# 2noise/ChatTTS

Measured on AMD Instinct MI355X. Metric: audio seconds/sec (RTF), batch=64 per GPU, higher is better.
Workload: dtype f32x3

## Files before the change

### chattts_amd/_lib.py

```python
from __future__ import annotations

import ctypes as C
import os

import torch

HERE = os.path.dirname(os.path.abspath(__file__))
LIB_PATH = os.environ.get("CTTS_LIB") or os.path.join(HERE, "csrc", "libchattts_amd.so")

F32, BF16 = 0, 1
P = C.c_void_p
PP = C.POINTER(C.c_void_p)


class GptWeights(C.Structure):
    _fields_ = [
        ("n_layers", C.c_int32), ("weight_dtype", C.c_int32), ("kv_dtype", C.c_int32), ("max_pos", C.c_int32),
        ("wqkv", PP), ("wo", PP), ("wgu", PP), ("wd", PP), ("ln1", PP), ("ln2", PP),
        ("norm", P), ("emb_code", P), ("heads", P), ("rope_cos", P), ("rope_sin", P),
        ("rms_eps", C.c_float),
        ("emb_text", P), ("head_text", P), ("n_text", C.c_int32),
        ("wqkv_pk", PP), ("wo_pk", PP), ("wgu_pk", PP), ("wd_pk", PP),
        ("heads_pk", P), ("head_text_pk", P),
        ("wo_hd", PP),
# ... 105 lines not shown
    "ctts_k_gemm": (C.c_int, [I32, P, P, P, I32, I32, I32, I32, I32, I32, I32, P, F, P, I32, P, P, I32, I32, I32, I32, I32, P]),
    "ctts_k_gemm_x3p": (C.c_int, [P, P, I32, I32, I32, I32, P, P, P, P, P, P]),
    "ctts_k_gemm_h1p": (C.c_int, [P, P, I32, I32, I32, I32, P, P, P, P, P, P]),
    "ctts_stream_create_cu_mask": (C.c_int, [I32, I32, I32, I32, P]),
    "ctts_stream_destroy": (C.c_int, [P]),
    "ctts_k_mlp_fused": (C.c_int, [P, P, P, I32, I32, P, P, P, P, I32, P]),
    "ctts_k_gemm_fast": (C.c_int, [P, I32, P, I32, I32, I32, P, F, I32, P, I32, P, I32, P, P]),
    "ctts_k_qkv_rope": (C.c_int, [P, P, I32, P, F, P, P, P, I32, P, P, I32, P, P, I32, P]),
    "ctts_k_gemm_dec": (C.c_int, [P, P, I32, I32, I32, P, P, F, I32, P, I32, P, I32, P, I32, P]),
    "ctts_k_gemm_dec32x": (C.c_int, [P, C.c_int64, P, C.c_int64, I32, I32, I32, P, P, I32, F, I32, P, I32, P, I32, P, C.c_int64, I32, P, I32, P, P, P]),
    "ctts_k_gemm_pre_x3": (C.c_int, [P, I32, P, P, I32, I32, I32, I32, I32, P, P, P, I32, P]),
    "ctts_k_dec32_last_variant": (C.c_char_p, []),
    "ctts_k_gemm_dec32": (C.c_int, [P, P, I32, I32, I32, P, P, I32, P, F, I32, P, I32, P, I32, P, I32, I32, I32, P]),
    "ctts_k_rows_prep": (C.c_int, [P, P, P, I32, P]),
    "ctts_k_rope_append": (C.c_int, [P, P, P, I32, I32, P, P, I32, P, P, I32, P]),
    "ctts_k_attention": (C.c_int, [P, P, P, I32, I32, P, I32, P, P, I32, P]),
    "ctts_k_attention_prefill": (C.c_int, [P, P, P, I32, P, I32, I32, P, I32, P]),
    "ctts_k_attention_dec": (C.c_int, [P, P, P, I32, P, P, P, I32, P, P, I32, P]),
    "ctts_k_attention_dec2": (C.c_int, [P, P, P, I32, I32, P, P, P, I32, I32, P]),
    "ctts_k_attention_cfg": (C.c_int, [I32, I32, I32]),
    "ctts_k_attention_heads_per_wg": (C.c_int, [I32]),
    "ctts_rccl_unique_id": (C.c_int, [P]),
    "ctts_rccl_comm_create": (C.c_int, [P, I32, P, I32]),
    "ctts_rccl_comm_destroy": (None, [P]),
    "ctts_broadcast_weights": (C.c_int, [P, P, I32, P, I32, P]),
    "ctts_k_attention_oproj": (C.c_int, [P, P, P, I32, P, P, P, I32, P, P, P, P, P, P]),
    "ctts_k_device_guard_probe": (C.c_int, [P, P, P, P, P]),
    "ctts_k_embed_codes": (C.c_int, [P, P, I32, P, P, I32, P]),
    "ctts_k_final_norm": (C.c_int, [P, I32, P, F, P, P, I32, P, I32, I32, P]),
    "ctts_k_sample": (C.c_int, [C.POINTER(GenState), P, P]),
# ... 44 lines not shown
```

### chattts_amd/csrc/capi.hip

```cpp
#include <hip/hip_runtime.h>
#include <dlfcn.h>
#include <stdarg.h>
#include <stdio.h>
#include <stdlib.h>
#include <string.h>
#include <algorithm>
#include <map>
#include <vector>

#include "../../include/chattts_amd.h"
#include "kernels.hpp"

static thread_local char g_err[512] = "";
int ctts_fail(const char* fmt, ...) {
  va_list ap;
  va_start(ap, fmt);
  vsnprintf(g_err, sizeof(g_err), fmt, ap);
  va_end(ap);
  return -1;
}
#define fail ctts_fail
#define CK(expr)                                                                                   \
  do {                                                                                             \
    hipError_t _e = (expr);                                                                        \
// ... 11 lines not shown
  std::vector<const void*> wqkv_pk, wo_pk, wgu_pk, wd_pk;
  std::vector<const void*> wo_hd;
  std::vector<const void*> wqkv_x3, wo_x3, wgu_x3, wd_x3;
  bool dec_x3 = false;
  bool qkv_att = false;
  bool att_oproj = false;
  bool dec_packed = false;
  bool dec_packed32 = false;
  bool heads_packed = false;
  int pf_mask = 0;
  int temporal_layers = 0;
  bool pre32_packed = true;
  bool embed_fold = false;
  bool pre_compact = true;
  bool pre_x3 = true;
  bool fnorm_fuse = true;
  std::vector<const float*> ln1, ln2;
  hipGraph_t graph = nullptr;
  hipGraphExec_t exec = nullptr;
  hipGraph_t graph_multi = nullptr;
  hipGraphExec_t exec_multi = nullptr;
  struct RowsGraph { hipGraph_t graph = nullptr, gm = nullptr; hipGraphExec_t exec = nullptr, exec_multi = nullptr; };
  std::map<int, RowsGraph> rows_graphs;
  int multi_steps = 1;
  int prof_tag = -1;
  int prof_max = 0;
  bool skip_finished = true;
  int n_cu = 0;
  int prof_stride = 1;
  int prof_seen = 0;
// ... 90 lines not shown
    g->wgu_x3.assign(w->wgu_x3, w->wgu_x3 + L);
    g->wd_x3.assign(w->wd_x3, w->wd_x3 + L);
    g->dec_x3 = true;
  }
  if (w->wo_hd && g->dec_packed) {
    g->wo_hd.assign(w->wo_hd, w->wo_hd + L);
    const char* e = getenv("CTTS_ATT_OPROJ");
    g->att_oproj = e && atoi(e) == 1;
  }
  { const char* e = getenv("CTTS_SKIP_FINISHED"); if (e && atoi(e) == 0) g->skip_finished = false; }
  { const char* e = getenv("CTTS_FNORM_FUSE"); if (e && atoi(e) == 0) g->fnorm_fuse = false; }
  { const char* e = getenv("CTTS_W_TEMPORAL_LAYERS"); if (e) g->temporal_layers = atoi(e); }
  { const char* e = getenv("CTTS_PF"); if (e) g->pf_mask = atoi(e); }
  { const char* e = getenv("CTTS_QKV_ATT"); g->qkv_att = e && atoi(e) == 1; }
  { const char* e = getenv("CTTS_PRE32_PACKED"); if (e && atoi(e) == 0) g->pre32_packed = false; }
  { const char* e = getenv("CTTS_PRE_X3"); if (e && atoi(e) == 0) g->pre_x3 = false; }
  { const char* e = getenv("CTTS_PRE_COMPACT"); if (e && atoi(e) == 0) g->pre_compact = false; }
  { const char* e = getenv("CTTS_EMBED_FOLD"); if (e) g->embed_fold = atoi(e) != 0; }
  {
    int dev = 0, cus = 0;
    const char* e = getenv("CTTS_ATT_SPLIT");
    if (e && atoi(e) == 1 && hipGetDevice(&dev) == hipSuccess &&
        hipDeviceGetAttribute(&cus, hipDeviceAttributeMultiprocessorCount, dev) == hipSuccess && cus > 0 && cus <= ATT_CUS_MAX)
      g->n_cu = cus;
  }
  *out = g;
  return 0;
}

extern "C" void ctts_gpt_graph_destroy(ctts_gpt* g) {
  if (!g) return;
// ... 255 lines not shown
    d.epi = D32_EPI_QKV_ROPE; d.C = ws.qkv; d.ldc = 3 * HID; d.desc = ws.desc; d.cos_t = g->w.rope_cos; d.sin_t = g->w.rope_sin;
    d.kc = (float*)kc; d.vc = (float*)vc; d.cmax = cmax;
    CK(launch_gemm_pre32(d, ws.rstd, st));
    CK(launch_attention(ws.qkv, kc, vc, kt, cmax, ws.aop32, 3, rm, M, st));
    d.Ap = ws.aop32; d.Wp = (const float*)g->wo_pk[l]; d.N = HID; d.norm_w = nullptr; d.epi = EPI_RES; d.C = ws.x; d.ldc = HID;
    d.res = ws.x; d.ldr = HID; d.Cp = ws.xp32; d.kch_out = HID / 16;
    CK(launch_gemm_pre32(d, nullptr, st));
    CK(launch_rows_rstd32(ws.x, HID, M, g->w.rms_eps, ws.rstd, st));
    d.Ap = ws.xp32; d.Wp = (const float*)g->wgu_pk[l]; d.N = INTER; d.norm_w = g->ln2[l]; d.epi = EPI_SILU_MUL; d.C = nullptr;
    d.res = nullptr; d.Cp = ws.actp32; d.kch_out = INTER / 16;
    CK(launch_gemm_pre32(d, ws.rstd, st));
    d.Ap = ws.actp32; d.Wp = (const float*)g->wd_pk[l]; d.N = HID; d.K = INTER; d.norm_w = nullptr; d.epi = EPI_RES;
    d.C = ws.x; d.ldc = HID; d.res = ws.x; d.ldr = HID; d.Cp = ws.xp32; d.kch_out = HID / 16;
    CK(launch_gemm_pre32(d, nullptr, st));
  }
  for (int l = 0; !fast && !packed32 && !pre32 && !x3 && l < g->w.n_layers; ++l) {
    void* kc = (char*)s->kcache + kv_layer * l;
    void* vc = (char*)s->vcache + kv_layer * l;
    GemmArgs a;
    memset(&a, 0, sizeof(a));
    a.taps = 1;
    a.n_active = nact;
    a.A = ws.x; a.lda = HID; a.W = g->wqkv[l]; a.C = ws.qkv; a.ldc = 3 * HID; a.M = M; a.N = 3 * HID; a.K = HID; a.wt = wt;
    a.epi = EPI_STORE; a.norm_w = g->ln1[l]; a.eps = g->w.rms_eps;
    if (pre_x3) { CK(launch_rows_rstd32(ws.x, HID, M, g->w.rms_eps, ws.rstd, st)); CK(launch_gemm_pre_x3(a, ws.rstd, st)); }
    else { Prof p(g, 1, st, prof_ok); CK(launch_gemm_skinny(a, st)); }
    { Prof p(g, 2, st, prof_ok); CK(launch_rope_append(ws.qkv, kc, vc, kt, cmax, g->w.rope_cos, g->w.rope_sin, rm, M, st)); }
    { Prof p(g, 3, st, prof_ok); CK(launch_attention(ws.qkv, kc, vc, kt, cmax, ws.ao, 0, rm, M, st)); }
    a.A = ws.ao; a.lda = HID; a.W = g->wo[l]; a.C = ws.x; a.ldc = HID; a.N = HID; a.K = HID; a.epi = EPI_RES; a.norm_w = nullptr;
    a.res = ws.x; a.ldr = HID;
    if (pre_x3) CK(launch_gemm_pre_x3(a, nullptr, st));
    else { Prof p(g, 4, st, prof_ok); CK(launch_gemm_skinny(a, st)); }
    a.A = ws.x; a.W = g->wgu[l]; a.C = ws.act; a.ldc = INTER; a.N = INTER; a.K = HID; a.epi = EPI_SILU_MUL; a.norm_w = g->ln2[l];
    a.res = nullptr;
    if (pre_x3) { CK(launch_rows_rstd32(ws.x, HID, M, g->w.rms_eps, ws.rstd, st)); CK(launch_gemm_pre_x3(a, ws.rstd, st)); }
    else { Prof p(g, 5, st, prof_ok); CK(launch_gemm_skinny(a, st)); }
    a.A = ws.act; a.lda = INTER; a.W = g->wd[l]; a.C = ws.x; a.ldc = HID; a.N = HID; a.K = INTER; a.epi = EPI_RES; a.norm_w = nullptr;
    a.res = ws.x; a.ldr = HID;
    if (pre_x3) CK(launch_gemm_pre_x3(a, nullptr, st));
    else { Prof p(g, 6, st, prof_ok); CK(launch_gemm_skinny(a, st)); }
  }
  if (!heads) return 0;
  if (fuse_fnorm) {
    const int nlog = s->infer_text ? g->w.n_text : NVQ * NAUDIO;
    Dec32Args d;
    memset(&d, 0, sizeof(d));
    d.Ap = x3 ? ws.hfinp : ws.xp32; d.Wp = s->infer_text ? g->w.head_text_pk : g->w.heads_pk; d.M = Bh; d.N = (nlog + 15) / 16 * 16; d.K = HID; d.n_active = nact;
    d.epi = EPI_STORE; d.C = ws.logits; d.ldc = nlog; d.n_cols = nlog;
    d.fnorm = 1; d.norm_w = g->w.norm; d.eps = g->w.rms_eps; d.desc = ws.desc; d.hid = s->hiddens; d.hid_cap = s->hid_cap ? s->hid_cap : s->max_new;
    d.T = s->T; d.prompt_len = s->prompt_len;
    Prof p(g, 8, st, prof_ok);
    CK(launch_gemm_dec32(d, st));
  } else {
  { Prof p(g, 7, st, prof_ok);
// ... 619 lines not shown
  return 0;
}
extern "C" int ctts_k_rope_append(float* qkv, void* kcache, void* vcache, int32_t kv_dtype, int32_t cmax, const float* cos_tab,
                                  const float* sin_tab, int32_t q_per_b, const int32_t* len, const int32_t* kv_start, int32_t M,
                                  void* stream) {
  GptRowMap rm{q_per_b, len, kv_start, nullptr, nullptr, nullptr, nullptr, nullptr, nullptr, 0, 0, 0};
  CK(launch_rope_append(qkv, kcache, vcache, kv_dtype, cmax, cos_tab, sin_tab, rm, M, (hipStream_t)stream));
  return 0;
}
extern "C" int ctts_k_attention(const float* qkv, const void* kcache, const void* vcache, int32_t kv_dtype, int32_t cmax, float* out,
                                int32_t q_per_b, const int32_t* len, const int32_t* kv_start, int32_t M, void* stream) {
  GptRowMap rm{q_per_b, len, kv_start, nullptr, nullptr, nullptr, nullptr, nullptr, nullptr, 0, 0, 0};
  CK(launch_attention(qkv, kcache, vcache, kv_dtype, cmax, out, 0, rm, M, (hipStream_t)stream));
  return 0;
}
extern "C" int ctts_k_attention_prefill(const float* qkv, const uint16_t* kcache, const uint16_t* vcache, int32_t cmax, float* out, int32_t q_per_b,
                                        int32_t slot0, const int32_t* kv_start, int32_t M, void* stream) {
  GptRowMap rm{q_per_b, nullptr, kv_start, nullptr, nullptr, nullptr, nullptr, nullptr, nullptr, 0, slot0, 0};
  CK(launch_attention(qkv, kcache, vcache, WT_BF16, cmax, out, 0, rm, M, (hipStream_t)stream));
  return 0;
}
extern "C" int ctts_k_attention_dec(const float* qkv, const uint16_t* kcache, const uint16_t* vcache, int32_t cmax, uint16_t* out_packed,
                                    const int32_t* desc, const int32_t* n_active, int32_t M, float* part, int32_t* cnt, int32_t n_cu,
                                    void* stream) {
  if (n_cu < 0 || n_cu > ATT_CUS_MAX) return fail("ctts_k_attention_dec: bad n_cu");
  GptRowMap rm{1, nullptr, nullptr, nullptr, n_active, nullptr, reinterpret_cast<const RowDesc*>(desc), part, cnt, n_cu, 0, 0};
  CK(launch_attention(qkv, kcache, vcache, WT_BF16, cmax, out_packed, 2, rm, M, (hipStream_t)stream));
  return 0;
}
extern "C" int ctts_k_attention_dec2(const float* qkv, const void* kcache, const void* vcache, int32_t kv_dtype, int32_t cmax, void* out_packed,
// ... 30 lines not shown
  CK(launch_embed_codes(emb_code, ids_buf, tcap, len, x, nullptr, nullptr, B, nullptr, nullptr, (hipStream_t)stream));
  return 0;
}
extern "C" int ctts_k_final_norm(const float* x, int32_t q_per_b, const float* w, float eps, float* hfin, float* hiddens,
                                 int32_t max_new, const int32_t* len, int32_t T, int32_t B, void* stream) {
  CK(launch_final_norm(x, q_per_b, w, eps, hfin, hiddens, max_new, len, T, B, nullptr, nullptr, nullptr, (hipStream_t)stream));
  return 0;
}
extern "C" int ctts_k_gemm_pre_x3(const float* A, int32_t lda, const float* W, float* C, int32_t ldc, int32_t M, int32_t N, int32_t K, int32_t epi,
                                  const float* norm_w, const float* rstd, const float* res, int32_t ldr, void* stream) {
  GemmArgs a;
  memset(&a, 0, sizeof(a));
  a.taps = 1; a.A = A; a.lda = lda; a.W = W; a.C = C; a.ldc = ldc; a.M = M; a.N = N; a.K = K; a.wt = WT_F32; a.epi = epi;
  a.norm_w = norm_w; a.res = res; a.ldr = ldr;
  CK(launch_gemm_pre_x3(a, rstd, (hipStream_t)stream));
  return 0;
}
extern "C" int ctts_k_sample(const ctts_gen_state* s, const float* logits, void* stream) {
  if (!s || !logits) return fail("ctts_k_sample: bad arguments");
  CK(launch_sample(make_sample_args(s, logits), (hipStream_t)stream));
  return 0;
}
extern "C" int ctts_k_sample_text(const ctts_gen_state* s, const float* logits, int32_t n_text, void* stream) {
  if (!s || !logits || n_text <= 0 || n_text > NTEXT_MAX) return fail("ctts_k_sample_text: bad arguments");
  CK(launch_sample_text(make_sample_args(s, logits), n_text, (hipStream_t)stream));
  return 0;
}
extern "C" int ctts_k_device_guard_probe(void* stream, int32_t* before, int32_t* stream_dev, int32_t* inside, int32_t* switched) {
  if (!before || !stream_dev || !inside || !switched) return fail("ctts_k_device_guard_probe: null argument");
  int b = -1, in = -1;
// ... 126 lines not shown
```

### chattts_amd/csrc/gpt.hip

```cpp
#include <stdlib.h>

#include "common.hpp"
#include "kernels.hpp"
#include "decode_dev.hpp"

#ifndef CTTS_QF_DELAY
#define CTTS_QF_DELAY 8
#endif
#ifndef CTTS_QF_PRE
#define CTTS_QF_PRE 1
#endif
#define HID 768
#define NHEAD 12
#define HDIM 64
#define NVQ 4
#define NAUDIO 626

__device__ __forceinline__ void row_to_b_slot(const GptRowMap& rm, int m, int& b, int& slot) {
  if (rm.q_per_b == 1) { b = rm.row_map ? rm.row_map[m] : m; slot = rm.len[b] - 1; }
  else { b = m / rm.q_per_b; slot = rm.slot0 + m - b * rm.q_per_b; if (rm.row_map) b = rm.row_map[b]; }
}
__device__ __forceinline__ bool row_absent(const int32_t* n_active, int m) { return n_active != nullptr && m >= *n_active; }

__device__ __forceinline__ void emit_row(float4 s, int t, float* __restrict__ x_row, uint16_t* __restrict__ xb_row,
// ... 231 lines not shown
template <> __device__ __forceinline__ void unpack16<float, 4>(const u128& r, float* f) {
  f[0] = __uint_as_float(r.x); f[1] = __uint_as_float(r.y); f[2] = __uint_as_float(r.z); f[3] = __uint_as_float(r.w);
}
template <> __device__ __forceinline__ void unpack16<bf16_t, 8>(const u128& r, float* f) {
  f[0] = __uint_as_float(r.x << 16); f[1] = __uint_as_float(r.x & 0xffff0000u);
  f[2] = __uint_as_float(r.y << 16); f[3] = __uint_as_float(r.y & 0xffff0000u);
  f[4] = __uint_as_float(r.z << 16); f[5] = __uint_as_float(r.z & 0xffff0000u);
  f[6] = __uint_as_float(r.w << 16); f[7] = __uint_as_float(r.w & 0xffff0000u);
}

template <typename OT> __device__ __forceinline__ size_t pko_off(int m, int c);
template <> __device__ __forceinline__ size_t pko_off<bf16_t>(int m, int c) { return pk_off(m, c, HID / 32); }
template <> __device__ __forceinline__ size_t pko_off<float>(int m, int c) { return pk32_off(m, c, HID / 16); }
struct x3p_t { uint16_t v; };
template <> __device__ __forceinline__ size_t pko_off<x3p_t>(int m, int c) { return pk_off(m, c, HID / 32); }
template <typename OT> __device__ __forceinline__ void store_out(OT* p, float v);
template <> __device__ __forceinline__ void store_out<x3p_t>(x3p_t* p, float v) { p->v = f32_to_bf16(v); }
template <typename OT> __device__ __forceinline__ void store_pko(OT* out, int m, int c, float v, size_t);
template <> __device__ __forceinline__ void store_pko<x3p_t>(x3p_t* out, int m, int c, float v, size_t plane) {
  uint16_t* p = reinterpret_cast<uint16_t*>(out) + pk_off(m, c, HID / 32);
  uint16_t h, l;
  x3_split(v, h, l);
  p[0] = h;
  p[plane] = l;
}
template <> __device__ __forceinline__ void store_out<float>(float* p, float v) { *p = v; }
template <> __device__ __forceinline__ void store_out<bf16_t>(bf16_t* p, float v) { *p = f32_to_bf16(v); }
template <> __device__ __forceinline__ void store_pko<float>(float* out, int m, int c, float v, size_t) { out[pko_off<float>(m, c)] = v; }
template <> __device__ __forceinline__ void store_pko<bf16_t>(bf16_t* out, int m, int c, float v, size_t) { out[pko_off<bf16_t>(m, c)] = f32_to_bf16(v); }

// ... 326 lines not shown
  u128 wv[OPJ ? 3 : 1][OPJ ? 8 : 1];
  if constexpr (OPJ) {
    const u128* wo = reinterpret_cast<const u128*>(rm.wo_h) + (size_t)h * 8 * HID + tid;
#pragma unroll
    for (int jc = 0; jc < 3; ++jc)
#pragma unroll
      for (int g8 = 0; g8 < 8; ++g8) wv[jc][g8] = load16(wo + (size_t)g8 * HID + 256 * jc);
    __builtin_amdgcn_sched_barrier(0);
  }
  lrun = groups_sum<LPK>(lrun, lane);
#pragma unroll
  for (int e = 0; e < DPL; ++e) acc[e] = groups_sum<LPK>(acc[e], lane);
  if (NW == 1) {
    if (kg == 0) {
      const float inv = 1.0f / lrun;
      OT* op = PKO ? out + pko_off<OT>(m, h * HDIM + dl * DPL) : out + (size_t)m * HID + h * HDIM + dl * DPL;
#pragma unroll
      for (int e = 0; e < DPL; ++e) store_out<OT>(op + e, acc[e] * inv);
    }
    return;
  }
  if (kg == 0) {
    if (dl == 0) { sm_m[wave] = mrun; sm_l[wave] = lrun; }
#pragma unroll
    for (int e = 0; e < DPL; ++e) sm_acc[wave][dl * DPL + e] = acc[e];
  }
  __syncthreads();
  if (tid < HDIM) {
    float M = -INFINITY;
#pragma unroll
    for (int w = 0; w < NW; ++w) M = fmaxf(M, sm_m[w]);
    float L = 0.f, o = 0.f;
#pragma unroll
// ... 511 lines not shown
    else if (nw_packed == 2)
      CTTS_LAUNCH_SMEM((attention_k<bf16_t, 2, bf16_t, true>), grid, dim3(128), att_lds, st, qkv, (const bf16_t*)kcache, (const bf16_t*)vcache, cmax, (bf16_t*)out, rm);
    else if (nw_packed == 8)
      CTTS_LAUNCH_SMEM((attention_k<bf16_t, 8, bf16_t, true>), grid, dim3(512), att_lds, st, qkv, (const bf16_t*)kcache, (const bf16_t*)vcache, cmax, (bf16_t*)out, rm);
    else if (nw_packed == 16)
      CTTS_LAUNCH_SMEM((attention_k<bf16_t, 16, bf16_t, true>), grid, dim3(1024), att_lds, st, qkv, (const bf16_t*)kcache, (const bf16_t*)vcache, cmax, (bf16_t*)out, rm);
    else if (att_nbuf == 3)
      CTTS_LAUNCH_SMEM((attention_k<bf16_t, 4, bf16_t, true, false, false, 3>), grid, dim3(256), att_lds, st, qkv, (const bf16_t*)kcache, (const bf16_t*)vcache, cmax, (bf16_t*)out, rm);
    else
      CTTS_LAUNCH_SMEM((attention_k<bf16_t, 4, bf16_t, true>), grid, dim3(256), att_lds, st, qkv, (const bf16_t*)kcache, (const bf16_t*)vcache, cmax, (bf16_t*)out, rm);
    return hipGetLastError();
  }
  if (out_bf16 == 3 && !decode) {
    if (kv_wt == WT_BF16) return hipErrorInvalidValue;
    CTTS_LAUNCH((attention_k<float, 1, float, true>), grid, dim3(64), st, qkv, (const float*)kcache, (const float*)vcache, cmax, (float*)out, rm);
    return hipGetLastError();
  }
  if (out_bf16 == 4) {
    if (!decode || kv_wt == WT_BF16 || rm.x3_plane == 0) return hipErrorInvalidValue;
    CTTS_LAUNCH_SMEM((attention_k<float, 4, x3p_t, true>), grid, dim3(256), att_lds, st, qkv, (const float*)kcache, (const float*)vcache, cmax, (x3p_t*)out, rm);
    return hipGetLastError();
  }
  if (out_bf16 == 3) {
    if (!decode || kv_wt == WT_BF16) return hipErrorInvalidValue;
    if (att_nbuf == 3)
      CTTS_LAUNCH_SMEM((attention_k<float, 4, float, true, false, false, 3>), grid, dim3(256), att_lds, st, qkv, (const float*)kcache, (const float*)vcache, cmax, (float*)out, rm);
    else
      CTTS_LAUNCH_SMEM((attention_k<float, 4, float, true>), grid, dim3(256), att_lds, st, qkv, (const float*)kcache, (const float*)vcache, cmax, (float*)out, rm);
    return hipGetLastError();
  }
// ... 844 lines not shown
```

### chattts_amd/csrc/kernels.hpp

```cpp
#pragma once
#include <hip/hip_runtime.h>
#include <hip/hip_ext.h>
#include <stdint.h>

#include "common.hpp"

extern thread_local hipEvent_t ctts_prof_start, ctts_prof_stop;
#define CTTS_LAUNCH(kern, grid, block, st, ...)                                                                   \
  do {                                                                                                            \
    if (ctts_prof_start) {                                                                                        \
      hipExtLaunchKernelGGL(kern, grid, block, 0, st, ctts_prof_start, ctts_prof_stop, 0, __VA_ARGS__);           \
      ctts_prof_start = nullptr; ctts_prof_stop = nullptr;                                                        \
    } else {                                                                                                      \
      hipLaunchKernelGGL(kern, grid, block, 0, st, __VA_ARGS__);                                                  \
    }                                                                                                             \
  } while (0)

#define CTTS_LAUNCH_SMEM(kern, grid, block, smem, st, ...)                                                        \
  do {                                                                                                            \
    if (ctts_prof_start) {                                                                                        \
      hipExtLaunchKernelGGL(kern, grid, block, smem, st, ctts_prof_start, ctts_prof_stop, 0, __VA_ARGS__);        \
      ctts_prof_start = nullptr; ctts_prof_stop = nullptr;                                                        \
    } else {                                                                                                      \
      hipLaunchKernelGGL(kern, grid, block, smem, st, __VA_ARGS__);                                               \
// ... 29 lines not shown
  int lda, ldc;
  int wt;
  int epi;
  const float* norm_w;
  float eps;
  const float* res; int ldr;
  const float* bias;
  const float* gamma;
  const int32_t* n_active;
  int taps, cin, frames, pad, dil;
  long long* dbg;
  const int2* seg;
};

hipError_t launch_gemm_skinny(const GemmArgs& a, hipStream_t st);
hipError_t launch_gemm_pre_x3(const GemmArgs& a, const float* rstd, hipStream_t st);

enum FastEpi { FEPI_STORE32 = 0, FEPI_RES = 1, FEPI_SILU = 2, FEPI_QKV_ROPE = 3 };
#define SSQ_PARTS 48
struct FastGemmArgs {
  const uint16_t* A; int lda;
  const uint16_t* W;
  int M, N, K;
  const float* ssq_in;
  float eps;
  int epi;
  float* C32; int ldc;
  uint16_t* Cb; int ldcb;
  float* ssq_out;
  int q_per_b; const int32_t* len; const int32_t* kv_start;
  const int32_t* row_map;
// ... 304 lines not shown
```

### chattts_amd/csrc/prefill32x.hip

```cpp
#include <stdlib.h>

#include "common.hpp"
#include "kernels.hpp"

namespace {

constexpr int XBK = 32, XLD = XBK + 8;
constexpr int XNT = 256;

typedef float xf2 __attribute__((ext_vector_type(2)));
typedef _Float16 xb2 __attribute__((ext_vector_type(2)));

__device__ __forceinline__ void split2(const float a, const float b, uint32_t& hi, uint32_t& lo) {
  const xf2 v = {a > 65504.0f ? 65504.0f : (a < -65504.0f ? -65504.0f : a), b > 65504.0f ? 65504.0f : (b < -65504.0f ? -65504.0f : b)};
  const xb2 h = __builtin_convertvector(v, xb2);
  hi = __builtin_bit_cast(uint32_t, h);
  const xf2 hf = __builtin_convertvector(h, xf2);
  const xb2 l = __builtin_convertvector((v - hf) * X3_LO_SCALE, xb2);
  lo = __builtin_bit_cast(uint32_t, l);
}
__device__ __forceinline__ void split4(const float4 v, ushort4& hi, ushort4& lo) {
  uint32_t h0, l0, h1, l1;
  split2(v.x, v.y, h0, l0);
  split2(v.z, v.w, h1, l1);
  hi = __builtin_bit_cast(ushort4, make_uint2(h0, h1));
  lo = __builtin_bit_cast(ushort4, make_uint2(l0, l1));
}

template <int EPI, int MBLK>
__global__ __launch_bounds__(XNT) void gemm_pre_x3_k(GemmArgs a, const float* __restrict__ rstd) {
  constexpr bool SILU = EPI == EPI_SILU_MUL;
  constexpr int BM = 64 * MBLK;
  constexpr int BN = 128;
  constexpr int BNO = SILU ? 64 : 128;
  __shared__ __attribute__((aligned(16))) uint16_t As[2][2][BM][XLD], Ws[2][2][BN][XLD];
  __shared__ float rstd_s[BM];

  const int tid = threadIdx.x, wave = tid >> 6, lane = tid & 63;
  const int wm = wave & 1, wn = wave >> 1;
  const int M = a.M, N = a.N, K = a.K;
  const int m0 = blockIdx.y * BM, n0 = blockIdx.x * BNO;
  const float* Wf = reinterpret_cast<const float*>(a.W);

  if (rstd != nullptr && tid < BM) rstd_s[tid] = rstd[min(m0 + tid, M - 1)];

// ... 81 lines not shown
#pragma unroll
    for (int j = 0; j < 2; ++j)
#pragma unroll
      for (int r = 0; r < 16; ++r) acc[i][j][r] += accx[i][j][r] * X3_LO_INV;
  const int cl = lane & 31;
#pragma unroll
  for (int i = 0; i < MBLK; ++i) {
#pragma unroll
    for (int r = 0; r < 16; ++r) {
      const int lrow = (wm * MBLK + i) * 32 + (r & 3) + 8 * (r >> 2) + 4 * (lane >> 5);
      const int row = m0 + lrow;
      if (row >= M) continue;
      const float rs = rstd != nullptr ? rstd_s[lrow] : 1.0f;
      if (EPI == EPI_SILU_MUL) {
        const int col = n0 + wn * 32 + cl;
        a.C[(size_t)row * a.ldc + col] = silu_f(acc[i][0][r] * rs) * (acc[i][1][r] * rs);
      } else {
#pragma unroll
        for (int j = 0; j < 2; ++j) {
          const int col = n0 + wn * 64 + j * 32 + cl;
          if (col >= N) continue;
          const float v = acc[i][j][r] * rs;
          a.C[(size_t)row * a.ldc + col] = (EPI == EPI_RES) ? a.res[(size_t)row * a.ldr + col] + v : v;
        }
      }
    }
  }
}

}

hipError_t launch_gemm_pre_x3(const GemmArgs& a, const float* rstd, hipStream_t st) {
  if (a.M <= 0 || a.N <= 0 || a.K <= 0 || (a.K % XBK) || (a.lda & 3) || !a.A || !a.W || !a.C || a.wt != WT_F32 || a.taps != 1) return hipErrorInvalidValue;
  if ((a.norm_w != nullptr) != (rstd != nullptr)) return hipErrorInvalidValue;
  if (a.epi == EPI_SILU_MUL ? (a.N % 64) != 0 : (a.N % 128) != 0) return hipErrorInvalidValue;
  if (a.epi == EPI_RES && !a.res) return hipErrorInvalidValue;
  const dim3 block(XNT);
  const int nx = a.epi == EPI_SILU_MUL ? a.N / 64 : a.N / 128;
  static int force_small = -1;
  if (force_small < 0) { const char* e = getenv("CTTS_PREX3_SMALL"); force_small = e ? atoi(e) : 0; }
  const bool small = force_small == 1 || (force_small != 2 && (long)nx * ((a.M + 127) / 128) < 1024);
  const dim3 grid(nx, small ? (a.M + 63) / 64 : (a.M + 127) / 128);
  switch (a.epi) {
    case EPI_SILU_MUL:
      if (small) CTTS_LAUNCH((gemm_pre_x3_k<EPI_SILU_MUL, 1>), grid, block, st, a, rstd); else CTTS_LAUNCH((gemm_pre_x3_k<EPI_SILU_MUL, 2>), grid, block, st, a, rstd);
      break;
    case EPI_RES:
      if (small) CTTS_LAUNCH((gemm_pre_x3_k<EPI_RES, 1>), grid, block, st, a, rstd); else CTTS_LAUNCH((gemm_pre_x3_k<EPI_RES, 2>), grid, block, st, a, rstd);
      break;
    case EPI_STORE:
      if (small) CTTS_LAUNCH((gemm_pre_x3_k<EPI_STORE, 1>), grid, block, st, a, rstd); else CTTS_LAUNCH((gemm_pre_x3_k<EPI_STORE, 2>), grid, block, st, a, rstd);
      break;
    default: return hipErrorInvalidValue;
  }
  return hipGetLastError();
}
```

### include/chattts_amd.h

```cpp
#ifndef CHATTTS_AMD_H
#define CHATTTS_AMD_H

#include <stddef.h>
#include <stdint.h>

#ifdef __cplusplus
extern "C" {
#endif

#define CTTS_F32 0
#define CTTS_BF16 1

typedef struct ctts_gpt ctts_gpt;
typedef struct ctts_codec ctts_codec;

const char* ctts_last_error(void);
int ctts_version(void);

typedef struct {
  int32_t n_layers;
  int32_t weight_dtype;
  int32_t kv_dtype;
  int32_t max_pos;
  const void* const* wqkv;
// ... 223 lines not shown
                    uint16_t* vcache, int32_t cmax, const float* cos_tab, const float* sin_tab, int32_t q_per_b, const int32_t* len,
                    const int32_t* kv_start, int32_t force_mb, void* stream);
int ctts_k_gemm_dec(const uint16_t* Ap, const uint16_t* Wp, int32_t M, int32_t N, int32_t K, const int32_t* n_active, const float* ssq_in,
                    float eps, int32_t epi, float* C32, int32_t ldc, uint16_t* Cp, int32_t kch_out, float* ssq_out, int32_t force_mb,
                    void* stream);
int ctts_k_gemm_dec32(const float* Ap, const float* Wp, int32_t M, int32_t N, int32_t K, const int32_t* n_active, const float* X, int32_t ldx,
                      const float* norm_w, float eps, int32_t epi, float* C, int32_t ldc, const float* res, int32_t ldr, float* Cp,
                      int32_t kch_out, int32_t force_mb, int32_t n_cols ,
                      void* stream);
int ctts_k_gemm_dec32x(const uint16_t* Ap, int64_t a_plane, const uint16_t* Wp, int64_t w_plane, int32_t M, int32_t N, int32_t K,
                       const int32_t* n_active, const float* X, int32_t ldx, float eps, int32_t epi, float* C, int32_t ldc, const float* res,
                       int32_t ldr, uint16_t* Cp, int64_t c_plane, int32_t kch_out, float* Cp32, int32_t force_mb, const float* ssq_in,
                       float* ssq_out, void* stream);
int ctts_k_gemm_pre_x3(const float* A, int32_t lda, const float* W, float* C, int32_t ldc, int32_t M, int32_t N, int32_t K, int32_t epi,
                       const float* norm_w, const float* rstd, const float* res, int32_t ldr, void* stream);
const char* ctts_k_dec32_last_variant(void);
int ctts_k_rows_prep(const float* x32, uint16_t* xb, float* ssq, int32_t M, void* stream);
int ctts_k_rope_append(float* qkv, void* kcache, void* vcache, int32_t kv_dtype, int32_t cmax, const float* cos_tab, const float* sin_tab,
                       int32_t q_per_b, const int32_t* len, const int32_t* kv_start, int32_t M, void* stream);
int ctts_k_attention(const float* qkv, const void* kcache, const void* vcache, int32_t kv_dtype, int32_t cmax, float* out,
                     int32_t q_per_b, const int32_t* len, const int32_t* kv_start, int32_t M, void* stream);
int ctts_k_attention_prefill(const float* qkv, const uint16_t* kcache, const uint16_t* vcache, int32_t cmax, float* out, int32_t q_per_b,
                             int32_t slot0, const int32_t* kv_start, int32_t M, void* stream);
int ctts_k_attention_dec(const float* qkv, const uint16_t* kcache, const uint16_t* vcache, int32_t cmax, uint16_t* out_packed,
                         const int32_t* desc, const int32_t* n_active, int32_t M, float* part, int32_t* cnt, int32_t n_cu, void* stream);
int ctts_k_attention_dec2(const float* qkv, const void* kcache, const void* vcache, int32_t kv_dtype, int32_t cmax, void* out_packed,
                          const int32_t* desc, const int32_t* n_active, int32_t covers_all, int32_t M, void* stream);
int ctts_k_attention_cfg(int32_t persist, int32_t workgroups, int32_t ring);
int ctts_k_attention_heads_per_wg(int32_t hpw);
int ctts_k_attention_oproj(const float* qkv, const uint16_t* kcache, const uint16_t* vcache, int32_t cmax, const uint16_t* wo_hd,
// ... 19 lines not shown
```

Baseline: 1048.

## Feed prefill O-proj and down-proj GEMMs from pre-split x3 fp16 planes

In the f32 prefill path, attention now writes its output directly as split hi/lo fp16 planes in packed tile layout, and the gate/up SiLU GEMM epilogue does the same for the activation. A new plane-input GEMM kernel (gemm_pre_x3p) then runs the O-projection and down-projection on the pre-packed weights with three MFMAs per tile. This removes the per-tile f32-to-x3 split of the A operand inside those GEMMs and reads half-width packed data. The cost is extra planar stores in producers, reuse of the aop32/actp32 workspaces as plane buffers, and a new, less tuned kernel. It is on by default and can be disabled with CTTS_PRE_X3=1.

Result: no change. 1050, median of 4 (+0.2%).

```diff
diff --git a/chattts_amd/_lib.py b/chattts_amd/_lib.py
--- a/chattts_amd/_lib.py
+++ b/chattts_amd/_lib.py
@@ -143,6 +143,9 @@
     "ctts_k_gemm_dec32": (C.c_int, [P, P, I32, I32, I32, P, P, I32, P, F, I32, P, I32, P, I32, P, I32, I32, I32, P]),
     "ctts_k_rows_prep": (C.c_int, [P, P, P, I32, P]),
     "ctts_k_rope_append": (C.c_int, [P, P, P, I32, I32, P, P, I32, P, P, I32, P]),
+    "ctts_k_gemm_pre_x3_silu_planes": (C.c_int, [P, I32, P, P, I32, I32, I32, I32, P, P, P, C.c_int64, P]),
+    "ctts_k_gemm_pre_x3p": (C.c_int, [P, C.c_int64, P, C.c_int64, P, I32, I32, I32, I32, P, I32, I32, P]),
+    "ctts_k_attention_x3p": (C.c_int, [P, P, P, I32, P, I32, P, P, I32, P]),
     "ctts_k_attention": (C.c_int, [P, P, P, I32, I32, P, I32, P, P, I32, P]),
     "ctts_k_attention_prefill": (C.c_int, [P, P, P, I32, P, I32, I32, P, I32, P]),
     "ctts_k_attention_dec": (C.c_int, [P, P, P, I32, P, P, P, I32, P, P, I32, P]),
diff --git a/chattts_amd/csrc/capi.hip b/chattts_amd/csrc/capi.hip
--- a/chattts_amd/csrc/capi.hip
+++ b/chattts_amd/csrc/capi.hip
@@ -49,6 +49,7 @@
   bool embed_fold = false;
   bool pre_compact = true;
   bool pre_x3 = true;
+  bool pre_x3_planes = true;
   bool fnorm_fuse = true;
   std::vector<const float*> ln1, ln2;
   hipGraph_t graph = nullptr;
@@ -169,7 +170,7 @@
   { const char* e = getenv("CTTS_PF"); if (e) g->pf_mask = atoi(e); }
   { const char* e = getenv("CTTS_QKV_ATT"); g->qkv_att = e && atoi(e) == 1; }
   { const char* e = getenv("CTTS_PRE32_PACKED"); if (e && atoi(e) == 0) g->pre32_packed = false; }
-  { const char* e = getenv("CTTS_PRE_X3"); if (e && atoi(e) == 0) g->pre_x3 = false; }
+  { const char* e = getenv("CTTS_PRE_X3"); if (e && atoi(e) == 0) g->pre_x3 = false; if (e && atoi(e) == 1) g->pre_x3_planes = false; }
   { const char* e = getenv("CTTS_PRE_COMPACT"); if (e && atoi(e) == 0) g->pre_compact = false; }
   { const char* e = getenv("CTTS_EMBED_FOLD"); if (e) g->embed_fold = atoi(e) != 0; }
   {
@@ -455,9 +456,13 @@
     d.C = ws.x; d.ldc = HID; d.res = ws.x; d.ldr = HID; d.Cp = ws.xp32; d.kch_out = HID / 16;
     CK(launch_gemm_pre32(d, nullptr, st));
   }
+  const bool pre_planes = pre_x3 && g->pre_x3_planes;
+  const size_t Mp16 = ((size_t)M + 15) / 16 * 16;
   for (int l = 0; !fast && !packed32 && !pre32 && !x3 && l < g->w.n_layers; ++l) {
     void* kc = (char*)s->kcache + kv_layer * l;
     void* vc = (char*)s->vcache + kv_layer * l;
+    uint16_t* aopx = reinterpret_cast<uint16_t*>(ws.aop32);
+    uint16_t* actx = reinterpret_cast<uint16_t*>(ws.actp32);
     GemmArgs a;
     memset(&a, 0, sizeof(a));
     a.taps = 1;
@@ -467,18 +472,25 @@
     if (pre_x3) { CK(launch_rows_rstd32(ws.x, HID, M, g->w.rms_eps, ws.rstd, st)); CK(launch_gemm_pre_x3(a, ws.rstd, st)); }
     else { Prof p(g, 1, st, prof_ok); CK(launch_gemm_skinny(a, st)); }
     { Prof p(g, 2, st, prof_ok); CK(launch_rope_append(ws.qkv, kc, vc, kt, cmax, g->w.rope_cos, g->w.rope_sin, rm, M, st)); }
-    { Prof p(g, 3, st, prof_ok); CK(launch_attention(ws.qkv, kc, vc, kt, cmax, ws.ao, 0, rm, M, st)); }
+    if (pre_planes) { rm.x3_plane = Mp16 * HID; Prof p(g, 3, st, prof_ok); CK(launch_attention(ws.qkv, kc, vc, kt, cmax, aopx, 4, rm, M, st)); }
+    else { Prof p(g, 3, st, prof_ok); CK(launch_attention(ws.qkv, kc, vc, kt, cmax, ws.ao, 0, rm, M, st)); }
     a.A = ws.ao; a.lda = HID; a.W = g->wo[l]; a.C = ws.x; a.ldc = HID; a.N = HID; a.K = HID; a.epi = EPI_RES; a.norm_w = nullptr;
     a.res = ws.x; a.ldr = HID;
-    if (pre_x3) CK(launch_gemm_pre_x3(a, nullptr, st));
+    PreX3pArgs xp;
+    memset(&xp, 0, sizeof(xp));
+    xp.res = ws.x; xp.ldr = HID; xp.C = ws.x; xp.ldc = HID; xp.M = M; xp.N = HID;
+    if (pre_planes) { xp.Ap = aopx; xp.a_plane = Mp16 * HID; xp.Wp = (const uint16_t*)g->wo_x3[l]; xp.w_plane = (size_t)HID * HID; xp.K = HID; CK(launch_gemm_pre_x3p(xp, st)); }
+    else if (pre_x3) CK(launch_gemm_pre_x3(a, nullptr, st));
     else { Prof p(g, 4, st, prof_ok); CK(launch_gemm_skinny(a, st)); }
     a.A = ws.x; a.W = g->wgu[l]; a.C = ws.act; a.ldc = INTER; a.N = INTER; a.K = HID; a.epi = EPI_SILU_MUL; a.norm_w = g->ln2[l];
     a.res = nullptr;
-    if (pre_x3) { CK(launch_rows_rstd32(ws.x, HID, M, g->w.rms_eps, ws.rstd, st)); CK(launch_gemm_pre_x3(a, ws.rstd, st)); }
+    if (pre_planes) { a.C = nullptr; CK(launch_rows_rstd32(ws.x, HID, M, g->w.rms_eps, ws.rstd, st)); CK(launch_gemm_pre_x3(a, ws.rstd, st, actx, Mp16 * INTER)); }
+    else if (pre_x3) { CK(launch_rows_rstd32(ws.x, HID, M, g->w.rms_eps, ws.rstd, st)); CK(launch_gemm_pre_x3(a, ws.rstd, st)); }
     else { Prof p(g, 5, st, prof_ok); CK(launch_gemm_skinny(a, st)); }
     a.A = ws.act; a.lda = INTER; a.W = g->wd[l]; a.C = ws.x; a.ldc = HID; a.N = HID; a.K = INTER; a.epi = EPI_RES; a.norm_w = nullptr;
     a.res = ws.x; a.ldr = HID;
-    if (pre_x3) CK(launch_gemm_pre_x3(a, nullptr, st));
+    if (pre_planes) { xp.Ap = actx; xp.a_plane = Mp16 * INTER; xp.Wp = (const uint16_t*)g->wd_x3[l]; xp.w_plane = (size_t)HID * INTER; xp.K = INTER; CK(launch_gemm_pre_x3p(xp, st)); }
+    else if (pre_x3) CK(launch_gemm_pre_x3(a, nullptr, st));
     else { Prof p(g, 6, st, prof_ok); CK(launch_gemm_skinny(a, st)); }
   }
   if (!heads) return 0;
@@ -1128,6 +1140,14 @@
   CK(launch_attention(qkv, kcache, vcache, kv_dtype, cmax, out, 0, rm, M, (hipStream_t)stream));
   return 0;
 }
+extern "C" int ctts_k_attention_x3p(const float* qkv, const float* kcache, const float* vcache, int32_t cmax, uint16_t* out_planes,
+                                    int32_t q_per_b, const int32_t* len, const int32_t* kv_start, int32_t M, void* stream) {
+  if (!out_planes || q_per_b <= 1 || M <= 0) return fail("ctts_k_attention_x3p: bad arguments");
+  GptRowMap rm{q_per_b, len, kv_start, nullptr, nullptr, nullptr, nullptr, nullptr, nullptr, 0, 0, 0};
+  rm.x3_plane = ((size_t)M + 15) / 16 * 16 * HID;
+  CK(launch_attention(qkv, kcache, vcache, WT_F32, cmax, out_planes, 4, rm, M, (hipStream_t)stream));
+  return 0;
+}
 extern "C" int ctts_k_attention_prefill(const float* qkv, const uint16_t* kcache, const uint16_t* vcache, int32_t cmax, float* out, int32_t q_per_b,
                                         int32_t slot0, const int32_t* kv_start, int32_t M, void* stream) {
   GptRowMap rm{q_per_b, nullptr, kv_start, nullptr, nullptr, nullptr, nullptr, nullptr, nullptr, 0, slot0, 0};
@@ -1188,6 +1208,26 @@
   a.taps = 1; a.A = A; a.lda = lda; a.W = W; a.C = C; a.ldc = ldc; a.M = M; a.N = N; a.K = K; a.wt = WT_F32; a.epi = epi;
   a.norm_w = norm_w; a.res = res; a.ldr = ldr;
   CK(launch_gemm_pre_x3(a, rstd, (hipStream_t)stream));
+  return 0;
+}
+extern "C" int ctts_k_gemm_pre_x3_silu_planes(const float* A, int32_t lda, const float* W, float* C, int32_t ldc, int32_t M, int32_t N, int32_t K,
+                                              const float* norm_w, const float* rstd, uint16_t* Cp, int64_t c_plane, void* stream) {
+  if (!Cp || c_plane <= 0) return fail("ctts_k_gemm_pre_x3_silu_planes: bad arguments");
+  GemmArgs a;
+  memset(&a, 0, sizeof(a));
+  a.taps = 1; a.A = A; a.lda = lda; a.W = W; a.C = C; a.ldc = ldc; a.M = M; a.N = N; a.K = K; a.wt = WT_F32; a.epi = EPI_SILU_MUL;
+  a.norm_w = norm_w;
+  CK(launch_gemm_pre_x3(a, rstd, (hipStream_t)stream, Cp, (size_t)c_plane));
+  return 0;
+}
+extern "C" int ctts_k_gemm_pre_x3p(const uint16_t* Ap, int64_t a_plane, const uint16_t* Wp, int64_t w_plane, float* C, int32_t ldc, int32_t M, int32_t N,
+                                   int32_t K, const float* res, int32_t ldr, int32_t tile, void* stream) {
+  if (a_plane <= 0 || w_plane <= 0 || tile < 0 || tile > 2) return fail("ctts_k_gemm_pre_x3p: bad arguments");
+  PreX3pArgs a;
+  memset(&a, 0, sizeof(a));
+  a.Ap = Ap; a.a_plane = (size_t)a_plane; a.Wp = Wp; a.w_plane = (size_t)w_plane; a.C = C; a.ldc = ldc; a.M = M; a.N = N; a.K = K;
+  a.res = res; a.ldr = ldr; a.tile = tile;
+  CK(launch_gemm_pre_x3p(a, (hipStream_t)stream));
   return 0;
 }
 extern "C" int ctts_k_sample(const ctts_gen_state* s, const float* logits, void* stream) {
diff --git a/chattts_amd/csrc/gpt.hip b/chattts_amd/csrc/gpt.hip
--- a/chattts_amd/csrc/gpt.hip
+++ b/chattts_amd/csrc/gpt.hip
@@ -269,6 +269,8 @@
 template <> __device__ __forceinline__ size_t pko_off<float>(int m, int c) { return pk32_off(m, c, HID / 16); }
 struct x3p_t { uint16_t v; };
 template <> __device__ __forceinline__ size_t pko_off<x3p_t>(int m, int c) { return pk_off(m, c, HID / 32); }
+template <typename OT> struct is_x3p { static constexpr bool value = false; };
+template <> struct is_x3p<x3p_t> { static constexpr bool value = true; };
 template <typename OT> __device__ __forceinline__ void store_out(OT* p, float v);
 template <> __device__ __forceinline__ void store_out<x3p_t>(x3p_t* p, float v) { p->v = f32_to_bf16(v); }
 template <typename OT> __device__ __forceinline__ void store_pko(OT* out, int m, int c, float v, size_t);
@@ -625,9 +627,14 @@
   if (NW == 1) {
     if (kg == 0) {
       const float inv = 1.0f / lrun;
-      OT* op = PKO ? out + pko_off<OT>(m, h * HDIM + dl * DPL) : out + (size_t)m * HID + h * HDIM + dl * DPL;
-#pragma unroll
-      for (int e = 0; e < DPL; ++e) store_out<OT>(op + e, acc[e] * inv);
+      if constexpr (PKO && is_x3p<OT>::value) {
+#pragma unroll
+        for (int e = 0; e < DPL; ++e) store_pko<OT>(out, m, h * HDIM + dl * DPL + e, acc[e] * inv, rm.x3_plane);
+      } else {
+        OT* op = PKO ? out + pko_off<OT>(m, h * HDIM + dl * DPL) : out + (size_t)m * HID + h * HDIM + dl * DPL;
+#pragma unroll
+        for (int e = 0; e < DPL; ++e) store_out<OT>(op + e, acc[e] * inv);
+      }
     }
     return;
   }
@@ -1169,6 +1176,11 @@
   if (out_bf16 == 3 && !decode) {
     if (kv_wt == WT_BF16) return hipErrorInvalidValue;
     CTTS_LAUNCH((attention_k<float, 1, float, true>), grid, dim3(64), st, qkv, (const float*)kcache, (const float*)vcache, cmax, (float*)out, rm);
+    return hipGetLastError();
+  }
+  if (out_bf16 == 4 && !decode) {
+    if (kv_wt == WT_BF16 || rm.x3_plane == 0) return hipErrorInvalidValue;
+    CTTS_LAUNCH((attention_k<float, 1, x3p_t, true>), grid, dim3(64), st, qkv, (const float*)kcache, (const float*)vcache, cmax, (x3p_t*)out, rm);
     return hipGetLastError();
   }
   if (out_bf16 == 4) {
diff --git a/chattts_amd/csrc/kernels.hpp b/chattts_amd/csrc/kernels.hpp
--- a/chattts_amd/csrc/kernels.hpp
+++ b/chattts_amd/csrc/kernels.hpp
@@ -67,7 +67,16 @@
 };
 
 hipError_t launch_gemm_skinny(const GemmArgs& a, hipStream_t st);
-hipError_t launch_gemm_pre_x3(const GemmArgs& a, const float* rstd, hipStream_t st);
+hipError_t launch_gemm_pre_x3(const GemmArgs& a, const float* rstd, hipStream_t st, uint16_t* cp = nullptr, size_t c_plane = 0);
+struct PreX3pArgs {
+  const uint16_t* Ap; size_t a_plane;
+  const uint16_t* Wp; size_t w_plane;
+  const float* res; int ldr;
+  float* C; int ldc;
+  int M, N, K;
+  int tile;
+};
+hipError_t launch_gemm_pre_x3p(const PreX3pArgs& a, hipStream_t st);
 
 enum FastEpi { FEPI_STORE32 = 0, FEPI_RES = 1, FEPI_SILU = 2, FEPI_QKV_ROPE = 3 };
 #define SSQ_PARTS 48
diff --git a/chattts_amd/csrc/prefill32x.hip b/chattts_amd/csrc/prefill32x.hip
--- a/chattts_amd/csrc/prefill32x.hip
+++ b/chattts_amd/csrc/prefill32x.hip
@@ -28,7 +28,7 @@
 }
 
 template <int EPI, int MBLK>
-__global__ __launch_bounds__(XNT) void gemm_pre_x3_k(GemmArgs a, const float* __restrict__ rstd) {
+__global__ __launch_bounds__(XNT) void gemm_pre_x3_k(GemmArgs a, const float* __restrict__ rstd, uint16_t* __restrict__ cp, const size_t c_plane) {
   constexpr bool SILU = EPI == EPI_SILU_MUL;
   constexpr int BM = 64 * MBLK;
   constexpr int BN = 128;
@@ -140,7 +140,15 @@
       const float rs = rstd != nullptr ? rstd_s[lrow] : 1.0f;
       if (EPI == EPI_SILU_MUL) {
         const int col = n0 + wn * 32 + cl;
-        a.C[(size_t)row * a.ldc + col] = silu_f(acc[i][0][r] * rs) * (acc[i][1][r] * rs);
+        const float v = silu_f(acc[i][0][r] * rs) * (acc[i][1][r] * rs);
+        if (a.C != nullptr) a.C[(size_t)row * a.ldc + col] = v;
+        if (cp != nullptr) {
+          uint16_t h, l;
+          x3_split(v, h, l);
+          uint16_t* at = cp + pk_off(row, col, N >> 5);
+          at[0] = h;
+          at[c_plane] = l;
+        }
       } else {
 #pragma unroll
         for (int j = 0; j < 2; ++j) {
@@ -154,10 +162,115 @@
   }
 }
 
-}
-
-hipError_t launch_gemm_pre_x3(const GemmArgs& a, const float* rstd, hipStream_t st) {
-  if (a.M <= 0 || a.N <= 0 || a.K <= 0 || (a.K % XBK) || (a.lda & 3) || !a.A || !a.W || !a.C || a.wt != WT_F32 || a.taps != 1) return hipErrorInvalidValue;
+template <int NBLK>
+__global__ __launch_bounds__(XNT) void gemm_pre_x3p_k(PreX3pArgs a) {
+  constexpr int TA = 4, TW = 4 * NBLK;
+  constexpr int CA = 2 * TA, CW = 2 * TW;
+  constexpr int PA = CA / 4, PW = CW / 4;
+  __shared__ __attribute__((aligned(16))) uint16_t As[2][CA][512], Ws[2][CW][512];
+
+  const int tid = threadIdx.x, wave = tid >> 6, lane = tid & 63;
+  const int wm = wave & 1, wn = wave >> 1;
+  const int M = a.M, N = a.N, KCH = a.K >> 5;
+  const int m0 = blockIdx.y * 64, n0 = blockIdx.x * (64 * NBLK);
+  const int mt_last = (M - 1) >> 4;
+
+  const u128* ap[PA];
+  const u128* wp[PW];
+#pragma unroll
+  for (int p = 0; p < PA; ++p) {
+    const int c = wave + 4 * p, plane = c / TA, mt = min((m0 >> 4) + c % TA, mt_last);
+    ap[p] = reinterpret_cast<const u128*>(a.Ap + plane * a.a_plane) + (size_t)mt * KCH * 64 + lane;
+  }
+#pragma unroll
+  for (int p = 0; p < PW; ++p) {
+    const int c = wave + 4 * p, plane = c / TW, nt = (n0 >> 4) + c % TW;
+    wp[p] = reinterpret_cast<const u128*>(a.Wp + plane * a.w_plane) + (size_t)nt * KCH * 64 + lane;
+  }
+  u128 ra[PA], rw[PW];
+#define XP_FETCH(KC)                                                                       \
+  do {                                                                                     \
+    _Pragma("unroll") for (int p = 0; p < PA; ++p) ra[p] = load16(ap[p] + (size_t)(KC) * 64); \
+    _Pragma("unroll") for (int p = 0; p < PW; ++p) rw[p] = load16(wp[p] + (size_t)(KC) * 64); \
+  } while (0)
+#define XP_STAGE(SB)                                                                                                  \
+  do {                                                                                                                \
+    _Pragma("unroll") for (int p = 0; p < PA; ++p) *reinterpret_cast<u128*>(&As[SB][wave + 4 * p][lane * 8]) = ra[p]; \
+    _Pragma("unroll") for (int p = 0; p < PW; ++p) *reinterpret_cast<u128*>(&Ws[SB][wave + 4 * p][lane * 8]) = rw[p]; \
+  } while (0)
+
+  f32x16 acc[NBLK], accx[NBLK];
+#pragma unroll
+  for (int j = 0; j < NBLK; ++j)
+#pragma unroll
+    for (int r = 0; r < 16; ++r) { acc[j][r] = 0.f; accx[j][r] = 0.f; }
+
+  XP_FETCH(0);
+  XP_STAGE(0);
+  if (1 < KCH) XP_FETCH(1);
+  __syncthreads();
+  const int ri = lane & 31, rt = ri >> 4, g2 = lane >> 5;
+  const int at = wm * 2 + rt;
+  int sb = 0;
+  for (int kc = 0; kc < KCH; ++kc) {
+    if (kc + 1 < KCH) XP_STAGE(sb ^ 1);
+    if (kc + 2 < KCH) XP_FETCH(kc + 2);
+#pragma unroll
+    for (int h = 0; h < 2; ++h) {
+      const int slot = ((2 * h + g2) * 16 + (ri & 15)) * 8;
+      const f16x8 ah = *reinterpret_cast<const f16x8*>(&As[sb][at][slot]);
+      const f16x8 al = *reinterpret_cast<const f16x8*>(&As[sb][TA + at][slot]);
+      f16x8 wh[NBLK], wl[NBLK];
+#pragma unroll
+      for (int j = 0; j < NBLK; ++j) {
+        wh[j] = *reinterpret_cast<const f16x8*>(&Ws[sb][(wn * NBLK + j) * 2 + rt][slot]);
+        wl[j] = *reinterpret_cast<const f16x8*>(&Ws[sb][TW + (wn * NBLK + j) * 2 + rt][slot]);
+      }
+#pragma unroll
+      for (int j = 0; j < NBLK; ++j) accx[j] = __builtin_amdgcn_mfma_f32_32x32x16_f16(al, wh[j], accx[j], 0, 0, 0);
+#pragma unroll
+      for (int j = 0; j < NBLK; ++j) accx[j] = __builtin_amdgcn_mfma_f32_32x32x16_f16(ah, wl[j], accx[j], 0, 0, 0);
+#pragma unroll
+      for (int j = 0; j < NBLK; ++j) acc[j] = __builtin_amdgcn_mfma_f32_32x32x16_f16(ah, wh[j], acc[j], 0, 0, 0);
+    }
+    __syncthreads();
+    sb ^= 1;
+  }
+#undef XP_FETCH
+#undef XP_STAGE
+
+  const int cl = lane & 31;
+#pragma unroll
+  for (int j = 0; j < NBLK; ++j) {
+    const int col = n0 + (wn * NBLK + j) * 32 + cl;
+#pragma unroll
+    for (int r = 0; r < 16; ++r) {
+      const int row = m0 + wm * 32 + (r & 3) + 8 * (r >> 2) + 4 * g2;
+      if (row >= M || col >= N) continue;
+      const float v = acc[j][r] + accx[j][r] * X3_LO_INV;
+      a.C[(size_t)row * a.ldc + col] = a.res[(size_t)row * a.ldr + col] + v;
+    }
+  }
+}
+
+}
+
+hipError_t launch_gemm_pre_x3p(const PreX3pArgs& a, hipStream_t st) {
+  if (a.M <= 0 || a.N <= 0 || a.K <= 0 || (a.K % XBK) || (a.N % 128) || !a.Ap || !a.Wp || !a.C || !a.res) return hipErrorInvalidValue;
+  if ((a.a_plane & 7) || (a.w_plane & 7) || a.a_plane < ((size_t)a.M + 15) / 16 * 16 * a.K || a.w_plane < (size_t)a.N * a.K) return hipErrorInvalidValue;
+  if ((reinterpret_cast<uintptr_t>(a.Ap) | reinterpret_cast<uintptr_t>(a.Wp)) & 15) return hipErrorInvalidValue;
+  static int env_tile = -1;
+  if (env_tile < 0) { const char* e = getenv("CTTS_PREX3P_TILE"); env_tile = e ? atoi(e) : 0; }
+  const int tile = a.tile ? a.tile : env_tile;
+  const int mt = (a.M + 63) / 64;
+  if (tile == 2) CTTS_LAUNCH((gemm_pre_x3p_k<2>), dim3(a.N / 128, mt), dim3(XNT), st, a);
+  else CTTS_LAUNCH((gemm_pre_x3p_k<1>), dim3(a.N / 64, mt), dim3(XNT), st, a);
+  return hipGetLastError();
+}
+
+hipError_t launch_gemm_pre_x3(const GemmArgs& a, const float* rstd, hipStream_t st, uint16_t* cp, size_t c_plane) {
+  if (a.M <= 0 || a.N <= 0 || a.K <= 0 || (a.K % XBK) || (a.lda & 3) || !a.A || !a.W || (!a.C && !cp) || a.wt != WT_F32 || a.taps != 1) return hipErrorInvalidValue;
+  if (cp != nullptr && (a.epi != EPI_SILU_MUL || (a.N & 31) || c_plane < ((size_t)a.M + 15) / 16 * 16 * a.N)) return hipErrorInvalidValue;
   if ((a.norm_w != nullptr) != (rstd != nullptr)) return hipErrorInvalidValue;
   if (a.epi == EPI_SILU_MUL ? (a.N % 64) != 0 : (a.N % 128) != 0) return hipErrorInvalidValue;
   if (a.epi == EPI_RES && !a.res) return hipErrorInvalidValue;
@@ -169,13 +282,13 @@
   const dim3 grid(nx, small ? (a.M + 63) / 64 : (a.M + 127) / 128);
   switch (a.epi) {
     case EPI_SILU_MUL:
-      if (small) CTTS_LAUNCH((gemm_pre_x3_k<EPI_SILU_MUL, 1>), grid, block, st, a, rstd); else CTTS_LAUNCH((gemm_pre_x3_k<EPI_SILU_MUL, 2>), grid, block, st, a, rstd);
+      if (small) CTTS_LAUNCH((gemm_pre_x3_k<EPI_SILU_MUL, 1>), grid, block, st, a, rstd, cp, c_plane); else CTTS_LAUNCH((gemm_pre_x3_k<EPI_SILU_MUL, 2>), grid, block, st, a, rstd, cp, c_plane);
       break;
     case EPI_RES:
-      if (small) CTTS_LAUNCH((gemm_pre_x3_k<EPI_RES, 1>), grid, block, st, a, rstd); else CTTS_LAUNCH((gemm_pre_x3_k<EPI_RES, 2>), grid, block, st, a, rstd);
+      if (small) CTTS_LAUNCH((gemm_pre_x3_k<EPI_RES, 1>), grid, block, st, a, rstd, cp, c_plane); else CTTS_LAUNCH((gemm_pre_x3_k<EPI_RES, 2>), grid, block, st, a, rstd, cp, c_plane);
       break;
     case EPI_STORE:
-      if (small) CTTS_LAUNCH((gemm_pre_x3_k<EPI_STORE, 1>), grid, block, st, a, rstd); else CTTS_LAUNCH((gemm_pre_x3_k<EPI_STORE, 2>), grid, block, st, a, rstd);
+      if (small) CTTS_LAUNCH((gemm_pre_x3_k<EPI_STORE, 1>), grid, block, st, a, rstd, cp, c_plane); else CTTS_LAUNCH((gemm_pre_x3_k<EPI_STORE, 2>), grid, block, st, a, rstd, cp, c_plane);
       break;
     default: return hipErrorInvalidValue;
   }
diff --git a/include/chattts_amd.h b/include/chattts_amd.h
--- a/include/chattts_amd.h
+++ b/include/chattts_amd.h
@@ -261,6 +261,12 @@
                        float* ssq_out, void* stream);
 int ctts_k_gemm_pre_x3(const float* A, int32_t lda, const float* W, float* C, int32_t ldc, int32_t M, int32_t N, int32_t K, int32_t epi,
                        const float* norm_w, const float* rstd, const float* res, int32_t ldr, void* stream);
+int ctts_k_gemm_pre_x3_silu_planes(const float* A, int32_t lda, const float* W, float* C, int32_t ldc, int32_t M, int32_t N, int32_t K,
+                                   const float* norm_w, const float* rstd, uint16_t* Cp, int64_t c_plane, void* stream);
+int ctts_k_gemm_pre_x3p(const uint16_t* Ap, int64_t a_plane, const uint16_t* Wp, int64_t w_plane, float* C, int32_t ldc, int32_t M, int32_t N,
+                        int32_t K, const float* res, int32_t ldr, int32_t tile, void* stream);
+int ctts_k_attention_x3p(const float* qkv, const float* kcache, const float* vcache, int32_t cmax, uint16_t* out_planes, int32_t q_per_b,
+                         const int32_t* len, const int32_t* kv_start, int32_t M, void* stream);
 const char* ctts_k_dec32_last_variant(void);
 int ctts_k_rows_prep(const float* x32, uint16_t* xb, float* ssq, int32_t M, void* stream);
 int ctts_k_rope_append(float* qkv, void* kcache, void* vcache, int32_t kv_dtype, int32_t cmax, const float* cos_tab, const float* sin_tab,
```
